# halide/Halide

Hardware: AMD Instinct MI355X
Metric: megapixels/sec local_laplacian 8-level fp32 4K (higher is better)
Workload: dtype f32; 1 GPU; apps/local_laplacian J=8 levels=8 alpha=1/7 beta=1, u16 RGB planar 3840x2160; distinct_frames_per_gpu=8, lut_cached=True, streams_per_gpu=4, frame_scheduling=4 frame-queue streams, boundary=C ABI local_laplacian(halide_buffer_t*,int32,float,float,halide_buffer_t*), rccl_ranks=1, parallelism=frames sharded over 1 GPU(s), no data-path collective

## Files before the change

halide_amd/csrc/hlmi_internal.h:

```cpp
#pragma once

#include <hip/hip_runtime.h>
#include <mutex>
#include <stdarg.h>
#include <stdint.h>
#include <stdio.h>
#include <string.h>
#include <type_traits>

#include "hlmi_pipelines.h"
#include "hlmi_runtime.h"

namespace hlmi {

int report(void *uc, int code, const char *fmt, ...) __attribute__((format(printf, 3, 4)));
int hip_failed(void *uc, hipError_t e, const char *what);

#define HLMI_HIP(uc, call)                                           \
    do {                                                             \
        hipError_t e__ = (call);                                     \
        if (e__ != hipSuccess) return ::hlmi::hip_failed(uc, e__, #call); \
    } while (0)

constexpr uint32_t type_abi(int code, int bits) { return (uint32_t)code | ((uint32_t)bits << 8); }
constexpr uint32_t T_U8 = type_abi(1, 8), T_U16 = type_abi(1, 16), T_I16 = type_abi(0, 16),
                   T_I32 = type_abi(0, 32), T_F32 = type_abi(2, 32);
inline uint32_t buf_type_abi(const halide_buffer_t *b) {
    uint32_t v;
    memcpy(&v, &b->type, 4);
    return v;
}
const char *type_name(uint32_t abi, char tmp[16]);

struct BufArg {
    const char *name;
    halide_buffer_t *buf;
    uint32_t type;
    int dims;
    bool is_output;
};

int check_not_null(void *uc, const BufArg *args, int n);
bool any_bounds_query(const BufArg *args, int n);
int check_type_and_dims(void *uc, const BufArg *args, int n);
int check_shape(void *uc, const BufArg &a);
int check_covers(void *uc, const BufArg &a, int d, int req_min, int req_extent);
int check_equal(void *uc, const char *what, int val, const char *expect_what, int expect);
int checks_done(void *uc);
void answer_query(halide_buffer_t *buf, const int *mins, const int *extents);

struct DeviceCtx {
    int device = -1;
    hipStream_t stream = nullptr;
    std::unique_lock<std::recursive_mutex> call_lock;
};
int acquire_device(void *uc, DeviceCtx *ctx, bool lock = true);
int get_workspace(void *uc, const DeviceCtx &ctx, size_t bytes, void **ptr);

int input_to_device(void *uc, const DeviceCtx &ctx, const BufArg &a);
int output_on_device(void *uc, const DeviceCtx &ctx, const BufArg &a);
void mark_output_written(halide_buffer_t *buf);
uint64_t buffer_version(const halide_buffer_t *buf);
int stream_cu_count(int device, hipStream_t stream);

inline bool buffer_is_real(const halide_buffer_t *b) { return !(b->host == nullptr && b->device == 0); }
inline bool buffer_has_shape(const halide_buffer_t *b) {
    for (int d = 0; d < b->dimensions; d++)
        if (b->dim[d].extent <= 0) return false;
    return b->dimensions > 0;
}
inline bool buffer_known(const halide_buffer_t *b) { return buffer_is_real(b) || buffer_has_shape(b); }

inline bool stream_is_special(hipStream_t s) { return s == nullptr || s == hipStreamLegacy || s == hipStreamPerThread; }
inline hipError_t record_done(hipEvent_t ev, hipStream_t producer) {
    if (stream_is_special(producer)) return hipStreamSynchronize(producer == hipStreamLegacy ? nullptr : producer);
    return hipEventRecord(ev, producer);
}
inline hipError_t wait_done(hipStream_t consumer, hipEvent_t ev) {
    if (stream_is_special(consumer)) return hipEventSynchronize(ev);
    return hipStreamWaitEvent(consumer, ev, 0);
}
inline hipStream_t event_stream(hipStream_t s) { return s == hipStreamLegacy ? nullptr : s; }

template<typename T>
inline T *dev_ptr(const halide_buffer_t *b) { return reinterpret_cast<T *>((uintptr_t)b->device); }

constexpr int DERIVED_SLOTS = 8, DERIVED_READERS = 4;
constexpr size_t DERIVED_KEY_BYTES = 96;
struct DerivedEntry {
    unsigned char key[DERIVED_KEY_BYTES];
    size_t key_bytes = 0;
    int device = -1;
    size_t bytes = 0;
    void *ptr = nullptr;
    hipStream_t stream = nullptr;
    hipEvent_t ready = nullptr;
    struct Reader {
        hipStream_t s = nullptr;
        hipEvent_t done = nullptr;
        bool live = false;
    } readers[DERIVED_READERS];
    bool overflow = false;
    int pins = 0;
    uint64_t used = 0;
};
struct DerivedCache {
    const int capacity;
    std::mutex mu;
    DerivedEntry slots[DERIVED_SLOTS];
    uint64_t clock = 0;
    explicit DerivedCache(int n) : capacity(n) {}
};
struct DerivedUse {
    void *ptr = nullptr;
    bool fill = true;
    void filled(hipStream_t s);
// ... 57 lines not shown
```

halide_amd/csrc/local_laplacian.hip:

```cpp
#include "hlmi_device_math.h"
#include "hlmi_internal.h"

#include <atomic>
#include <mutex>
#include <optional>
#include <stdlib.h>
#include <string.h>
#include <type_traits>

using namespace hlmi;

namespace {

constexpr int J = 8;
constexpr int MAX_K = 32;
constexpr int STRIP = 126;
constexpr int KCH = 8;
constexpr int D0_THREADS = 256;

struct Level {
    int lox, loy;
    int w, h;
    int ws;
    size_t ps;
// ... 604 lines not shown
    prep_row(rd, p1);
    load_row(rc, 2 * T0 + 3);
    load_row(rd, 2 * T0 + 4);
    LL_PROBE_T(pt2);
    for (int T = T0; T <= T1; T += 2) {
        const bool first = EXCH && T == T0;
        step(std::integral_constant<int, 0>{}, T, p0, p1, p2, p3, a, b, a2, b2, first && publish ? pub_mine : nullptr);
        step(std::integral_constant<int, 1>{}, T + 1, p2, p3, p0, p1, a2, b2, a, b,
             first && publish ? pub_mine + (KCH + 1) * 64 : nullptr);
        if (first) __syncthreads();
#if HLMI_LL_PROBE
        if (first) { LL_PROBE_T(pt3); pr_3 = pt3; }
#endif
    }
    LL_PROBE_T(pt4);
    LL_PROBE_ADD(0, pt1 - pt0); LL_PROBE_ADD(1, 1); LL_PROBE_ADD(2, pt2 - pt1); LL_PROBE_ADD(3, pr_3 - pt2);
    LL_PROBE_ADD(16, pr_a - pr_a0); LL_PROBE_ADD(17, pr_a0 - pt1);
    LL_PROBE_ADD(4, pt4 - pt2); LL_PROBE_ADD(5, (T1 - T0 + 1)); LL_PROBE_ADD(6, pt4 - pt0);
    if (EXCH && !self_halo) {
        float *d2 = p.g2 + (size_t)(B - p.loy2) * p.ws2 + off2;
#pragma unroll
        for (int k = 0; k <= KCH; k++) {
            const float2 sa = st2[(2 * k) * 64], sb = st2[(2 * k + 1) * 64];
            const float2 c = pub_next[k * 64], d = pub_next[(KCH + 1 + k) * 64];
            const float rx = dev::mad(3.0f, sb.x + c.x, sa.x) + d.x, ry = dev::mad(3.0f, sb.y + c.y, sa.y) + d.y;
            float o;
            if (ODD1) {
                const float nx = lane_next(rx), ny = lane_next(ry);
                o = down4_tail(rx, ry, nx, ny);
            } else {
                const float py = lane_prev(ry), nx = lane_next(rx);
                o = down4_tail(py, rx, ry, nx);
            }
            if (st2_ok) d2[(size_t)k * p.ps2] = o;
        }
    }
    };
    if (edge_wave) walk(std::true_type{});
    else walk(std::false_type{});
}

struct D01EArgs {
    D01Args d;
    float *outl0;
    int oy0, oh;
    unsigned nsx_magic;
};
typedef float f2 __attribute__((ext_vector_type(2)));
__device__ __forceinline__ f2 f2s(float v) { return f2{v, v}; }
__device__ __forceinline__ f2 fma2(f2 a, f2 b, f2 c) { return __builtin_elementwise_fma(a, b, c); }
__device__ __forceinline__ f2 mad_2(f2 a, f2 b, f2 c) { return dev::CANON_FMA ? fma2(a, b, c) : a * b + c; }
__device__ __forceinline__ f2 mad2_2(f2 a, f2 b, f2 c, f2 d) { return dev::CANON_FMA ? fma2(a, b, c * d) : a * b + c * d; }

template<bool ODD0, bool ODD1, bool B1, bool EXCH, bool NT>
__global__ __launch_bounds__(D0_THREADS, 2) void ll_down01e(D01EArgs pe, Geometry gm, Levels lev) {
    const D01Args &p = pe.d;
    LL_RESIDENCY(0);
    extern __shared__ float slut[];
    for (int i = threadIdx.x; i <= 2 * gm.half; i += D0_THREADS) slut[i] = p.lut_g[i];
    __syncthreads();
    const int wave = __builtin_amdgcn_readfirstlane(threadIdx.x >> 6);
    const int lane = threadIdx.x & 63;
    int sx, A, B;
    bool self_halo = true;
    bool publish = false;
    if (EXCH) {
        const int wg = xcd_block();
        const int gy = pe.nsx_magic ? (int)__umulhi((unsigned)wg, pe.nsx_magic) : wg;
        sx = wg - gy * p.nsx;
        const int GA = p.loy2 + gy * p.rows_base + min(gy, p.rows_rem);
        const int GB = GA + p.rows_base + (gy < p.rows_rem ? 1 : 0) - 1;
        const int n = (GB - GA + 1 + 1 + 3) >> 2;
        A = GA + wave * n, B = min(A + n - 1, GB);
        if (A > GB) {
            __syncthreads();
            return;
        }
        self_halo = !(wave < 3 && A + n <= GB);
        publish = wave > 0;
    } else {
        const int unit = xcd_block() * (D0_THREADS / 64) + wave;
        if (unit >= p.nunits) return;
        sx = p.nsy_magic ? (int)__umulhi((unsigned)unit, p.nsy_magic) : unit;
        const int sy = unit - sx * p.nsy;
        A = p.loy2 + sy * p.rows_base + min(sy, p.rows_rem);
        B = A + p.rows_base + (sy < p.rows_rem ? 1 : 0) - 1;
    }
    const int P = p.Pbase + 2 * p.S2 * sx + 2 * lane;
    const int q0 = ODD0 ? 2 * P - 1 : 2 * P - 2;
    const int iw = gm.ix1 - gm.ix0 + 1, ih = gm.iy1 - gm.iy0;
    const QuadSel qs = quad_sel(q0 - gm.ix0, iw);
    int xo[4];
#pragma unroll
    for (int i = 0; i < 4; i++) xo[i] = qs.oq + qs.sel[i];
    const bool edge_wave = __any(!qs.plain);
    const int T0 = 2 * A - 1, T1 = self_halo ? 2 * B + 2 : 2 * B;
    const int Ts0 = max(EXCH ? 2 * A - 1 : 2 * A, p.loy1), Ts1 = min(EXCH ? 2 * B : 2 * B + 1, p.loy1 + p.h1 - 1);
    const int off1 = P - p.so1;
    const bool st1_ok = lane < p.S2 && off1 >= 0 && off1 < p.w1;
    const int X2 = ODD1 ? (P + 1) >> 1 : P >> 1;
    const int off2 = X2 - p.so2;
    const bool st2_ok = (ODD1 ? lane < p.S2 : (lane >= 1 && lane <= p.S2)) && off2 >= 0 && off2 < p.w2;
    const bool em_ok = lane >= 1 && lane <= p.S2 && q0 >= gm.ix0 && q0 + 3 <= gm.ix1;
    float *const em_col = pe.outl0 + (q0 - gm.ix0);
    f2 *st2 = reinterpret_cast<f2 *>(slut + ((2 * gm.half + 2) & ~1)) + wave * D01_STATE + lane;
    f2 *pub_all = reinterpret_cast<f2 *>(slut + ((2 * gm.half + 2) & ~1)) + (D0_THREADS / 64) * D01_STATE + lane;
    f2 *pub_mine = pub_all + (wave - 1) * D01_STATE, *pub_next = pub_all + wave * D01_STATE;
    const int lbase = gm.half - 256 * (KCH - 1);
    float level[KCH];
#pragma unroll
    for (int kk = 0; kk < KCH; kk++) {
        level[kk] = lev.v[kk];
        asm volatile("" : "+v"(level[kk]));
    }
    auto walk = [&](auto edge_tag) {
    constexpr bool EDGE = decltype(edge_tag)::value;
    auto load_row = [&](Raw &r, int y_abs) {
        const uint16_t *rp = p.in + (long)(dev::clampi(y_abs - gm.iy0, 0, ih)) * p.in_sy;
        load_raw<true, NT>(r, rp, p.co0, p.co1, p.co2, qs.oq, xo);
    };
    auto u16s = [&](const ushort4 &c, uint16_t (&o)[4]) {
        const uint2 w = __builtin_bit_cast(uint2, c);
        o[0] = (uint16_t)(w.x & 0xffffu), o[1] = (uint16_t)(w.x >> 16);
        o[2] = (uint16_t)(w.y & 0xffffu), o[3] = (uint16_t)(w.y >> 16);
    };
    struct Row {
        f2 g[2];
        int l[4];
    };
    auto prep_row = [&](const Raw &r, Row &o) {
        uint16_t rr[4], gg[4], bb[4];
        u16s(r.c0, rr), u16s(r.c1, gg), u16s(r.c2, bb);
        constexpr float s = (float)(1.0 / 65535.0);
        constexpr float C0 = (float)((double)s * (double)0.299f), C1 = (float)((double)s * (double)0.587f),
                        C2 = (float)((double)s * (double)0.114f);
#pragma unroll
        for (int h = 0; h < 2; h++) {
            const f2 fr = {(float)rr[h], (float)rr[h + 2]}, fg = {(float)gg[h], (float)gg[h + 2]}, fb = {(float)bb[h], (float)bb[h + 2]};
            o.g[h] = mad_2(fb, f2s(C2), mad2_2(fr, f2s(C0), fg, f2s(C1)));
        }
        if (EDGE) {
            const float g0 = o.g[0].x, g1v = o.g[1].x, g2v = o.g[0].y, g3 = o.g[1].y;
            o.g[0].x = pick4(g0, g1v, g2v, g3, qs.sel[0]), o.g[1].x = pick4(g0, g1v, g2v, g3, qs.sel[1]);
            o.g[0].y = pick4(g0, g1v, g2v, g3, qs.sel[2]), o.g[1].y = pick4(g0, g1v, g2v, g3, qs.sel[3]);
        }
#pragma unroll
        for (int h = 0; h < 2; h++) {
            const f2 t = (o.g[h] * gm.Km1) * 256.0f;
            o.l[h] = (min((int)t.x, gm.half) + lbase) * 4;
            o.l[h + 2] = (min((int)t.y, gm.half) + lbase) * 4;
        }
#pragma unroll
        for (int i = 0; i < 4; i++) asm volatile("" : "+v"(o.l[i]));
    };
    auto lut_issue = [&](int kk, const Row &r0, const Row &r1, f2 (&dst)[4]) {
        auto rd = [&](int l) {
            return *reinterpret_cast<const float *>(reinterpret_cast<const char *>(slut) + l + 1024 * (KCH - 1 - kk));
        };
        dst[0].x = rd(r0.l[0]), dst[1].x = rd(r0.l[1]), dst[0].y = rd(r0.l[2]), dst[1].y = rd(r0.l[3]);
        dst[2].x = rd(r1.l[0]), dst[3].x = rd(r1.l[1]), dst[2].y = rd(r1.l[2]), dst[3].y = rd(r1.l[3]);
// ... 236 lines not shown
            em_wait(eg[0], after3), eo[0] = em_arith(n0, 0, eg[0], row_odd);
            __builtin_amdgcn_sched_barrier(0);
            em_gather(n1, 0, rowP, rowT, fg[0]);
            __builtin_amdgcn_sched_barrier(0);
            em_wait(eg[1], after3), eo[1] = em_arith(n0, 1, eg[1], row_odd);
            __builtin_amdgcn_sched_barrier(0);
            em_gather(n1, 1, rowP, rowT, fg[1]);
            __builtin_amdgcn_sched_barrier(0);
            em_wait(eg[2], after3), eo[2] = em_arith(n0, 2, eg[2], row_odd);
            __builtin_amdgcn_sched_barrier(0);
            em_gather(n1, 2, rowP, rowT, fg[2]);
            __builtin_amdgcn_sched_barrier(0);
            em_wait(eg[3], after3), eo[3] = em_arith(n0, 3, eg[3], row_odd);
            __builtin_amdgcn_sched_barrier(0);
            em_gather(n1, 3, rowP, rowT, fg[3]);
            __builtin_amdgcn_sched_barrier(0);
            em_wait(fg[0], after3), ee[0] = em_arith(n1, 0, fg[0], row_even);
            em_wait(fg[1], after2), ee[1] = em_arith(n1, 1, fg[1], row_even);
            em_wait(fg[2], after1), ee[2] = em_arith(n1, 2, fg[2], row_even);
            em_wait(fg[3], after0), ee[3] = em_arith(n1, 3, fg[3], row_even);
        }
        asm volatile("" ::: "memory");
        __builtin_amdgcn_sched_barrier(0);
        LL_PROBE_T(ps2);
        prep_row(rc, n0);
        prep_row(rd, n1);
        __builtin_amdgcn_sched_barrier(0);
        if (st1_row && st1_ok) {
            float *drow = p.g1 + (size_t)(T - p.loy1) * p.ws1 + off1;
            *reinterpret_cast<float2 *>(drow) = s0;
            *reinterpret_cast<float2 *>(drow + p.ps1) = s1;
            *reinterpret_cast<f2 *>(drow + (size_t)KCH * p.ps1) = sK;
        }
        if (em_rows) {
            emit_store(2 * T - 1, eo);
            emit_store(2 * T, ee);
        }
        __builtin_amdgcn_sched_barrier(0);
        if (T + 1 < T1) {
            load_row(rc, 2 * T + 5);
            load_row(rd, 2 * T + 6);
        }
        __builtin_amdgcn_sched_barrier(0);
#if HLMI_LL_PROBE
        LL_PROBE_T(ps3);
        pr_planes += ps1 - ps0, pr_emit += ps2 - ps1, pr_prep += ps3 - ps2, pr_steps += 1;
#endif
    };
    Row p0, p1, p2, p3;
    prep_row(rc, p0);
    prep_row(rd, p1);
    load_row(rc, 2 * T0 + 3);
    load_row(rd, 2 * T0 + 4);
    for (int T = T0; T <= T1; T += 2) {
        const bool first = EXCH && T == T0;
        step(std::integral_constant<int, 0>{}, T, p0, p1, p2, p3, a, b, a2, b2, first && publish ? pub_mine : nullptr);
        step(std::integral_constant<int, 1>{}, T + 1, p2, p3, p0, p1, a2, b2, a, b, first && publish ? pub_mine + 64 : nullptr);
        if (first) __syncthreads();
    }
#if HLMI_LL_PROBE
    LL_PROBE_T(pe1);
#endif
    if (EXCH && !self_halo) {
        float *d2 = p.g2 + (size_t)(B - p.loy2) * p.ws2 + off2;
#pragma unroll
        for (int k = 0; k <= KCH; k++) {
            const f2 sa = st2[(2 * k) * 64], sb = st2[(2 * k + 1) * 64];
            const f2 c = pub_next[(2 * k) * 64], d = pub_next[(2 * k + 1) * 64];
            const f2 r = mad_2(f2s(3.0f), sb + c, sa) + d;
            float o;
            if (ODD1) {
                const float nx = lane_next(r.x), ny = lane_next(r.y);
                o = down4_tail(r.x, r.y, nx, ny);
            } else {
                const float py = lane_prev(r.y), nx = lane_next(r.x);
                o = down4_tail(py, r.x, r.y, nx);
            }
            if (st2_ok) d2[(size_t)k * p.ps2] = o;
        }
        {
            float eo[4], ee[4];
            emit_row(p2, pub_next, st2 + 64, eo, row_odd);
            emit_row(p3, st2 + 64, pub_next, ee, row_even);
            emit_store(4 * B + 1, eo);
            emit_store(4 * B + 2, ee);
        }
    }
#if HLMI_LL_PROBE
    LL_PROBE_T(pe2);
    LL_PROBE_ADD(27, __builtin_readcyclecounter() - pc0);
    LL_PROBE_ADD(28, pe2 - pe0);
    LL_PROBE_ADD(20, pr_planes); LL_PROBE_ADD(21, pr_emit); LL_PROBE_ADD(22, pr_prep); LL_PROBE_ADD(23, pr_steps);
    LL_PROBE_ADD(24, 1); LL_PROBE_ADD(25, pe1 - pe0); LL_PROBE_ADD(26, pe2 - pe1);
#endif
    };
    if (edge_wave) walk(std::true_type{});
    else walk(std::false_type{});
}

struct StripArgs {
    const float *src;
    int slox, sloy, sw, sh, sws;
    size_t sps;
    float *dst;
    int Xs, dloy, dw, dh, dws;
    size_t dps;
    int nsx, nsy, nunits;
};
template<bool ODD>
__device__ __forceinline__ void down_strip_unit(const StripArgs &a, int unit, int lane) {
    const int sy = unit % a.nsy, rest = unit / a.nsy, sx = rest % a.nsx, plane = rest / a.nsx;
    const int off = STRIP * sx + 2 * lane;
    const int P = a.Xs + off;
    const QuadSel qs = quad_sel((ODD ? 2 * P - 1 : 2 * P - 2) - a.slox, a.sw);
    const bool edge_wave = __any(!qs.plain);
    const bool store_ok = (lane < 63) && (off < a.dw);
    const int t0 = (int)((long)sy * a.dh / a.nsy), t1 = (int)((long)(sy + 1) * a.dh / a.nsy) - 1;
    const float *sp = a.src + (size_t)plane * a.sps + qs.oq;
    float *dp = a.dst + (size_t)plane * a.dps + off;
    auto row = [&](int y_abs) -> float4 {
        float4 v = *reinterpret_cast<const float4 *>(sp + (size_t)dev::clampi(y_abs - a.sloy, 0, a.sh - 1) * a.sws);
        if (edge_wave) {
            v = make_float4(pick4(v.x, v.y, v.z, v.w, qs.sel[0]), pick4(v.x, v.y, v.z, v.w, qs.sel[1]),
                            pick4(v.x, v.y, v.z, v.w, qs.sel[2]), pick4(v.x, v.y, v.z, v.w, qs.sel[3]));
        }
        return v;
    };
    const int T0 = a.dloy + t0;
    float4 ra = row(2 * T0 - 1), rb = row(2 * T0), rc = row(2 * T0 + 1), rd = row(2 * T0 + 2);
    for (int t = t0; t <= t1; t++) {
        const int T = a.dloy + t;
        float4 nc = rc, nd = rd;
        if (t < t1) {
            nc = row(2 * T + 3);
            nd = row(2 * T + 4);
        }
// ... 881 lines not shown
const halide_scalar_value_t est_one = [] { halide_scalar_value_t v{}; v.u.f32 = 1.0f; return v; }();
const halide_type_t ty_u16 = {(decltype(halide_type_t::code))1, 16, 0};
const halide_type_t ty_i32 = {(decltype(halide_type_t::code))0, 32, 0};
const halide_type_t ty_f32 = {(decltype(halide_type_t::code))2, 32, 0};
const halide_filter_argument_t ll_args[5] = {
    {"input", halide_argument_kind_input_buffer, 3, ty_u16, nullptr, nullptr, nullptr, nullptr, buf_est},
    {"levels", halide_argument_kind_input_scalar, 0, ty_i32, nullptr, nullptr, nullptr, &est_levels, nullptr},
    {"alpha", halide_argument_kind_input_scalar, 0, ty_f32, nullptr, nullptr, nullptr, &est_one, nullptr},
    {"beta", halide_argument_kind_input_scalar, 0, ty_f32, nullptr, nullptr, nullptr, &est_one, nullptr},
    {"output", halide_argument_kind_output_buffer, 3, ty_u16, nullptr, nullptr, nullptr, nullptr, buf_est},
};
const halide_filter_metadata_t ll_md = {1, 5, ll_args, kTargetString, "local_laplacian"};

struct LlSwitches {
    std::optional<int> fuse_from, upchain_from, ru, units0, no_vec, emit, nt, fuse_up2, d01_exch, d01_pad_lds, no_lut_cache;
};
LlSwitches ll_switches() {
    auto get = [](const char *name) -> std::optional<int> {
        const char *e = getenv(name);
        if (e && *e) return atoi(e);
        return std::nullopt;
    };
    LlSwitches s;
    s.fuse_from = get("HLMI_LL_FUSE_FROM"), s.upchain_from = get("HLMI_LL_UPCHAIN_FROM");
    s.ru = get("HLMI_LL_RU"), s.units0 = get("HLMI_LL_UNITS0"), s.no_vec = get("HLMI_LL_NO_VEC");
    s.emit = get("HLMI_LL_EMIT"), s.nt = get("HLMI_LL_NT"), s.fuse_up2 = get("HLMI_LL_FUSE_UP2");
    s.d01_exch = get("HLMI_LL_D01_EXCH"), s.d01_pad_lds = get("HLMI_LL_D01_PAD_LDS"), s.no_lut_cache = get("HLMI_LL_NO_LUT_CACHE");
    return s;
}

int dev_clamp_ru(int ru) { return ru < 1 ? 1 : (ru > 300 ? 300 : ru); }

struct PairGeom {
    int S2;
    int Pbase;
    int nsx;
};
struct LlPlan {
    Geometry gm;
    Level lv[J];
    size_t off_g[J], off_out[J], off_l0, ws_floats;
    Up0Args u0;
    int nlut;
    int S, SU;
    int up_low;
    bool lut_cache;
    bool lut_lds;
    bool vec_frame;
    bool vec_in;
    bool b1;
    bool fast, fuse1, fuse2, emit, nt;
    bool d01;
    bool strip2;
    struct { PairGeom pg; bool exch; int nsy, nunits; size_t lds; } d0;
    struct { PairGeom pg; int nsy, nunits; } s2;
    int units_strip;
    size_t up0_lds;
};

struct LlBuffers {
    float *lut, *outl0;
    float *g[J], *outg[J];
};

PairGeom pair_geom(const Level &d, const Level &e) {
    PairGeom g;
    g.S2 = (d.odd || e.odd) ? 62 : 61;
    const int lim = e.odd ? 2 * e.lox - 1 : 2 * e.lox - 2;
    g.Pbase = min(d.lox, lim);
    const int hi1 = d.lox + d.w - 1, hi2 = e.lox + e.w - 1;
    const int x2_first = e.odd ? (g.Pbase + 1) / 2 + 0 : g.Pbase / 2 + 1;
    g.nsx = max((hi2 - x2_first + g.S2) / g.S2, (hi1 - g.Pbase + 2 * g.S2) / (2 * g.S2));
    return g;
}

void ll_plan(LlPlan &pl, const halide_buffer_t *input, const halide_buffer_t *output, int levels, float beta, const LlSwitches &sw,
             int stream_cus, int device_cus) {
    Up0Args &p = pl.u0;
    const int ow = p.ow = output->dim[0].extent, oh = p.oh = output->dim[1].extent, nc = p.nc = output->dim[2].extent;
    Geometry &gm = pl.gm;
    gm.K = levels;
    gm.half = (levels - 1) * 256;
    gm.Km1 = (float)(levels - 1);
    gm.inv_Km1 = 1.0f / gm.Km1;
    gm.ix0 = input->dim[0].min, gm.ix1 = gm.ix0 + input->dim[0].extent - 1;
    gm.iy0 = input->dim[1].min, gm.iy1 = gm.iy0 + input->dim[1].extent - 1;
    const int ic0 = input->dim[2].min, ic1 = ic0 + input->dim[2].extent - 1, iw = gm.ix1 - gm.ix0 + 1;

    Level *lv = pl.lv;
    int lox = gm.ix0, hix = gm.ix1, loy = gm.iy0, hiy = gm.iy1, so = gm.ix0;
    int rx0 = output->dim[0].min, rx1 = rx0 + ow - 1, ry0 = output->dim[1].min, ry1 = ry0 + oh - 1;
    size_t ws_floats = (size_t)(2 * gm.half + 1 + 63) & ~(size_t)63;
    for (int j = 0; j < J; j++) {
        Level &L = lv[j];
        L.lox = so, L.loy = loy, L.w = hix - so + 1, L.h = hiy - loy + 1;
        L.ws = (L.w + 3) & ~3;
        L.ps = ((size_t)L.ws * L.h + 3) & ~(size_t)3;
        L.rx0 = rx0, L.rx1 = rx1, L.ry0 = ry0, L.ry1 = ry1;
        if (j >= 1) {
            pl.off_g[j] = ws_floats;
            ws_floats += ((size_t)(levels + 1) * L.ps + 63) & ~(size_t)63;
            pl.off_out[j] = ws_floats;
            ws_floats += (L.ps + 63) & ~(size_t)63;
        }
        const bool odd = (so & 1) != 0;
        const int par = odd ? (floor_div(so + 1, 2) & 1) : ((floor_div(so, 2) + 1) & 1);
        lox = floor_div(lox - 2, 2), hix = floor_div(hix + 2, 2);
        loy = floor_div(loy - 2, 2), hiy = floor_div(hiy + 2, 2);
        so = lox - ((lox - par) & 1);
        if (j + 1 < J) {
            lv[j + 1].odd = odd;
            lv[j + 1].nsx = (hix - so + 1 + STRIP - 1) / STRIP;
        }
        rx0 = floor_div(rx0 - 1, 2), rx1 = floor_div(rx1 + 1, 2);
        ry0 = floor_div(ry0 - 1, 2), ry1 = floor_div(ry1 + 1, 2);
    }
    p.in = dev_ptr<uint16_t>(input), p.out = dev_ptr<uint16_t>(output);
    const uintptr_t din = (uintptr_t)p.in, dout = (uintptr_t)p.out;
    const long in_sy = p.in_sy = input->dim[1].stride, in_sc = input->dim[2].stride;
    const long out_sy = p.out_sy = output->dim[1].stride, out_sc = p.out_sc = output->dim[2].stride;
    p.ox0 = output->dim[0].min, p.oy0 = output->dim[1].min;
    p.beta = beta, pl.b1 = (beta == 1.0f);
    const int oc0 = output->dim[2].min;
    bool same = (nc == 3);
    for (int ch = 0; ch < 3; ch++) {
        p.gco[ch] = (long)((ch < ic0 ? ic0 : (ch > ic1 ? ic1 : ch)) - ic0) * in_sc;
        p.cco[ch] = ch < nc ? (long)(oc0 + ch - ic0) * in_sc : 0;
        if (p.cco[ch] != p.gco[ch]) same = false;
    }
    p.same_ch = same ? 1 : 0;
// ... 10 lines not shown
        const int v = sw.upchain_from.value_or(S == 4 ? 3 : 0);
        return (v >= 1 && v <= J - 2) ? v : S;
    }();
    const bool partitioned = stream_cus < device_cus;
    bool vec_frame = (din % 4 == 0) && (dout % 4 == 0) && in_sy % 2 == 0 && out_sy % 2 == 0 && out_sc % 2 == 0 &&
                     ((p.ox0 - gm.ix0) % 2 == 0) && !sw.no_vec.value_or(0);
    for (int ch = 0; ch < 3; ch++) vec_frame = vec_frame && p.gco[ch] % 2 == 0 && p.cco[ch] % 2 == 0;
    pl.vec_frame = vec_frame;
    const bool vec_in = pl.vec_in = (din % 8 == 0) && in_sy % 4 == 0 && p.gco[0] % 4 == 0 && p.gco[1] % 4 == 0 && p.gco[2] % 4 == 0 &&
                                    iw % 4 == 0 && !sw.no_vec.value_or(0);
    const bool fast = pl.fast = vec_frame && same && nc == 3 && (ow & 1) == 0 && (p.ox0 & 1) == 0 &&
                                (double)(levels + 1) * (4.0 * (double)lv[1].ps) < 4.0e9;
    const bool fuse1 = pl.fuse1 = fast && SU >= 2;
    const bool d01 = pl.d01 = levels == KCH && lut_lds && vec_in;
    const bool emit = pl.emit = d01 && fast && fuse1 && lv[1].ws < (1 << 24) && sw.emit.value_or(1);
    const int RU = p.RU = dev_clamp_ru(sw.ru.value_or(emit ? (partitioned ? 32 : 8) : fuse1 ? (partitioned ? 32 : 16) : 8));
    pl.nt = sw.nt.value_or(partitioned ? 1 : 0) != 0;
    pl.fuse2 = emit && SU >= 3 && SU < J && sw.fuse_up2.value_or(1);
    pl.up_low = fuse1 ? (pl.fuse2 ? 3 : 2) : 1;
    pl.strip2 = d01 && S == 4;

    pl.off_l0 = ws_floats;
    if (emit) ws_floats += ((size_t)iw * (size_t)oh + 63) & ~(size_t)63;
    pl.ws_floats = ws_floats;

    constexpr int WPB = D0_THREADS / 64;
    if (!d01) {
        const Level &d = lv[1];
        const int target = sw.units0.value_or(8 * device_cus);
        pl.d0.nsy = max(1, min(max(target / d.nsx, (d.h + 63) / 64), max(1, d.h / 2)));
        pl.d0.nunits = d.nsx * pl.d0.nsy;
        pl.d0.lds = (lut_lds ? sizeof(float) * ((nlut + 1) & ~1) : 0) + sizeof(float2) * D0_THREADS * (KCH + 1);
    } else {
        const Level &e = lv[2];
        const PairGeom pg = pl.d0.pg = pair_geom(lv[1], e);
        const int target2 = sw.units0.value_or(emit && partitioned ? 10 * stream_cus : 8 * device_cus);
        bool exch = sw.d01_exch.value_or(1) != 0;
        int nwy = 0;
        auto ceil_div = [](int x, int y) { return (x + y - 1) / y; };
        if (exch) {
            const int nwy_max = max(1, target2 / (WPB * pg.nsx));
            const int n = max(2, (ceil_div(e.h, nwy_max) + 1 + 3) / 4);
            nwy = ceil_div(e.h, 4 * n - 1);
            exch = e.h / nwy >= 4;
        }
        pl.d0.exch = exch;
        if (exch) {
            pl.d0.nsy = nwy;
            pl.d0.nunits = pg.nsx * nwy * WPB;
        } else {
            pl.d0.nsy = max(1, min(max(target2 / pg.nsx, (e.h + 31) / 32), e.h));
            pl.d0.nunits = pg.nsx * pl.d0.nsy;
        }
        size_t sh2 = sizeof(float) * ((nlut + 1) & ~1) + sizeof(float2) * D01_STATE * (WPB + (exch ? WPB - 1 : 0));
        const int pad = sw.d01_pad_lds.value_or(emit && partitioned ? -1 : 0);
        constexpr size_t kHalfCuLds = 160 * 1024 / 2;
        if (pad < 0) sh2 = max(sh2, kHalfCuLds + 2048);
        else sh2 += (size_t)pad;
        pl.d0.lds = sh2;
    }
    if (pl.strip2) {
        pl.s2.pg = pair_geom(lv[3], lv[4]);
        pl.s2.nsy = (lv[4].h + S2_RPU - 1) / S2_RPU;
        pl.s2.nunits = (levels + 1) * pl.s2.pg.nsx * pl.s2.nsy;
    }
    pl.units_strip = 16 * device_cus;
    pl.up0_lds = emit   ? sizeof(float) * ((size_t)U0_TS * (RU + 2) + (size_t)U0H_T2 * (RU / 2 + 4))
                 : fast ? lut_sh + (fuse1 ? ((lut_lds && (nlut & 1)) ? 4 : 0) + sizeof(float) * U0_TS * (RU + 2) : 0)
                        : lut_sh;
}

struct LlLastCall {
    LlPlan pl;
    LlBuffers b;
    hipStream_t stream;
    bool out1_pending;
    bool out2_pending;
};
thread_local LlLastCall t_dbg = {};

StripArgs strip_args(const LlPlan &pl, const LlBuffers &b, int j) {
    const Level &sl = pl.lv[j], &d = pl.lv[j + 1];
    const int cols = d.nsx * (pl.gm.K + 1);
    StripArgs a;
    a.src = b.g[j], a.slox = sl.lox, a.sloy = sl.loy, a.sw = sl.w, a.sh = sl.h, a.sws = sl.ws, a.sps = sl.ps;
    a.dst = b.g[j + 1], a.Xs = d.lox, a.dloy = d.loy, a.dw = d.w, a.dh = d.h, a.dws = d.ws, a.dps = d.ps;
    a.nsx = d.nsx;
    a.nsy = max(1, min(max(pl.units_strip / cols, (d.h + 31) / 32), max(1, d.h / 2)));
    a.nunits = cols * a.nsy;
    return a;
}
CoarseArgs coarse_args(const LlPlan &pl, const LlBuffers &b, int from) {
    CoarseArgs ca;
    for (int dl = 0; from + dl < J; dl++) {
        const Level &L = pl.lv[from + dl];
        DevLevel &D = ca.lv[dl];
        D.g = b.g[from + dl], D.out = b.outg[from + dl], D.lox = L.lox, D.loy = L.loy, D.w = L.w, D.h = L.h, D.ws = L.ws, D.ps = (unsigned)L.ps;
        D.rx0 = L.rx0, D.ry0 = L.ry0, D.rw = L.rx1 - L.rx0 + 1, D.rh = L.ry1 - L.ry0 + 1;
    }
    ca.K = pl.gm.K, ca.Km1 = pl.gm.Km1;
    return ca;
}
UpArgs up_args(const LlPlan &pl, const LlBuffers &b, int j) {
    const Level &a = pl.lv[j], &c = pl.lv[j + 1];
    UpArgs u;
    u.g = b.g[j], u.ws = a.ws, u.ps = a.ps, u.lox = a.lox, u.loy = a.loy, u.gc = b.g[j + 1], u.outc = b.outg[j + 1], u.cws = c.ws, u.cps = c.ps;
    u.clox = c.lox, u.cloy = c.loy, u.rx0 = a.rx0, u.ry0 = a.ry0, u.rw = a.rx1 - a.rx0 + 1, u.rh = a.ry1 - a.ry0 + 1;
    u.K = pl.gm.K, u.Km1 = pl.gm.Km1, u.out = b.outg[j];
    return u;
}

// ... 4 lines not shown
static_assert(sizeof(LutKey) <= DERIVED_KEY_BYTES, "key does not fit an entry");
DerivedCache g_luts(8);


int ll_stage_table(void *uc, const DeviceCtx &ctx, const LlPlan &pl, float alpha, LlBuffers &b, DerivedUse &use) {
    const int nlut = pl.nlut;
    LutKey key;
    memset(&key, 0, sizeof key);
    key.device = ctx.device, key.levels = pl.gm.K;
    memcpy(&key.alpha_bits, &alpha, 4);
    int r = derived_acquire(uc, ctx, g_luts, &key, sizeof key, sizeof(float) * ((size_t)nlut + 64), pl.lut_cache, &use);
    if (r) return r;
    if (use.ptr) b.lut = (float *)use.ptr;
    if (use.fill) {
        HLMI_LAUNCH(uc, "ll_remap_lut", ctx.stream, ll_remap_lut, dim3((nlut + 255) / 256), dim3(256), 0, b.lut, pl.gm.half, alpha);
        use.filled(ctx.stream);
    }
    return 0;
}

int ll_stage_down0(void *uc, const LlPlan &pl, const LlBuffers &b, hipStream_t st) {
    const Geometry &gm = pl.gm;
    const Up0Args &f = pl.u0;
    const Level &d = pl.lv[1], &e = pl.lv[2];
    const int levels = gm.K, iw = gm.ix1 - gm.ix0 + 1;
    Levels lev;
    for (int k = 0; k < MAX_K; k++) lev.v[k] = (float)k * gm.inv_Km1;
    constexpr int WPB = D0_THREADS / 64;
    dim3 block(D0_THREADS);
    const double d0_bytes = 6.0 * iw * (gm.iy1 - gm.iy0 + 1) + 4.0 * (levels + 1) * d.w * d.h;
    if (!pl.d01) {
        dim3 grid((pl.d0.nunits + WPB - 1) / WPB);
        timing_note_bytes(d0_bytes);
        return with_flags([&](auto O, auto V, auto L, auto B) -> int {
            HLMI_LAUNCH(uc, "ll_down0", st, (ll_down0<O.value, V.value, L.value, B.value>), grid, block, pl.d0.lds, f.in, f.in_sy,
                        f.gco[0], f.gco[1], f.gco[2], gm, lev, f.beta, b.lut, b.g[1], d.lox, d.loy, d.w, d.h, d.ws, d.ps, d.nsx,
                        pl.d0.nsy, pl.d0.nunits);
            return 0;
        }, d.odd, pl.vec_in, pl.lut_lds, pl.b1);
    }
    D01Args a;
    a.in = f.in, a.in_sy = f.in_sy, a.co0 = f.gco[0], a.co1 = f.gco[1], a.co2 = f.gco[2], a.beta = f.beta, a.lut_g = b.lut;
    a.g1 = b.g[1], a.so1 = d.lox, a.loy1 = d.loy, a.w1 = d.w, a.h1 = d.h, a.ws1 = d.ws, a.ps1 = d.ps;
    a.g2 = b.g[2], a.so2 = e.lox, a.loy2 = e.loy, a.w2 = e.w, a.h2 = e.h, a.ws2 = e.ws, a.ps2 = e.ps;
    a.S2 = pl.d0.pg.S2, a.Pbase = pl.d0.pg.Pbase, a.nsx = pl.d0.pg.nsx, a.nsy = pl.d0.nsy, a.nunits = pl.d0.nunits;
    a.nsy_magic = a.nsy == 1 ? 0u : (unsigned)((1ull << 32) / (unsigned)a.nsy + 1ull);
    a.rows_base = e.h / a.nsy, a.rows_rem = e.h % a.nsy;
    dim3 grid((a.nunits + WPB - 1) / WPB);
    if (pl.emit) {
        timing_note_bytes(6.0 * iw * (gm.iy1 - gm.iy0 + 1) + 4.0 * iw * f.oh + 4.0 * 3.0 * d.w * d.h + 4.0 * (levels + 1) * e.w * e.h);
        D01EArgs ae;
        ae.d = a, ae.outl0 = b.outl0, ae.oy0 = f.oy0, ae.oh = f.oh;
        ae.nsx_magic = a.nsx == 1 ? 0u : (unsigned)((1ull << 32) / (unsigned)a.nsx + 1ull);
        return with_flags([&](auto O0, auto O1, auto B, auto EX, auto NT) -> int {
            HLMI_LAUNCH(uc, "ll_down01", st, (ll_down01e<O0.value, O1.value, B.value, EX.value, NT.value>), grid, block, pl.d0.lds, ae, gm, lev);
            return 0;
        }, d.odd, e.odd, pl.b1, pl.d0.exch, pl.nt);
    }
    timing_note_bytes(d0_bytes + 4.0 * (levels + 1) * e.w * e.h);
    return with_flags([&](auto O0, auto O1, auto B, auto EX) -> int {
        HLMI_LAUNCH(uc, "ll_down01", st, (ll_down01f<O0.value, O1.value, B.value, EX.value>), grid, block, pl.d0.lds, a, gm, lev);
        return 0;
    }, d.odd, e.odd, pl.b1, pl.d0.exch);
}

int ll_stage_down_rest(void *uc, const LlPlan &pl, const LlBuffers &b, hipStream_t st) {
    const Level *lv = pl.lv;
    const int levels = pl.gm.K, S = pl.S;
    if (pl.strip2) {
        const Level &sl = lv[2], &d = lv[3], &e = lv[4];
        Strip2Args a;
        a.src = b.g[2], a.slox = sl.lox, a.sloy = sl.loy, a.sw = sl.w, a.sh = sl.h, a.sws = sl.ws, a.sps = sl.ps;
        a.g1 = b.g[3], a.so1 = d.lox, a.loy1 = d.loy, a.w1 = d.w, a.h1 = d.h, a.ws1 = d.ws, a.ps1 = d.ps;
        a.g2 = b.g[4], a.so2 = e.lox, a.loy2 = e.loy, a.w2 = e.w, a.h2 = e.h, a.ws2 = e.ws, a.ps2 = e.ps;
        a.S2 = pl.s2.pg.S2, a.Pbase = pl.s2.pg.Pbase, a.nsx = pl.s2.pg.nsx, a.nsy = pl.s2.nsy, a.nunits = pl.s2.nunits;
        timing_note_bytes(4.0 * (levels + 1) * ((double)sl.w * sl.h + (double)d.w * d.h + (double)e.w * e.h));
        dim3 grid((a.nunits + 3) / 4), block(256);
        if (int r = with_flags([&](auto O0, auto O1) -> int {
                HLMI_LAUNCH(uc, "ll_down_strip2:2", st, (ll_down_strip2<O0.value, O1.value>), grid, block, 0, a);
                return 0;
            }, d.odd, e.odd)) return r;
    }
    for (int j = 1; j + 1 < J; j++) {
        if (pl.strip2 && (j == 2 || j == 3)) continue;
        if (j == S) {
            const CoarseArgs ca = coarse_args(pl, b, S);
            long total = 0;
            for (int dl = 1; S + dl < J; dl++) total += (long)(levels + 1) * lv[S + dl].w * lv[S + dl].h;
            const int ntx = (lv[J - 1].w + DM_T - 1) / DM_T, nty = (lv[J - 1].h + DM_T - 1) / DM_T;
            dim3 grid((unsigned)(ntx * nty * (levels + 1))), block(256);
            char nm[32];
            snprintf(nm, sizeof nm, "ll_down_multi:%d", S);
            timing_note_bytes(4.0 * ((double)(levels + 1) * lv[S].w * lv[S].h + (double)total));
            if (J - 1 - S == 4) HLMI_LAUNCH(uc, nm, st, (ll_down_multi<4>), grid, block, 0, ca, ntx, nty);
            else if (J - 1 - S == 3) HLMI_LAUNCH(uc, nm, st, (ll_down_multi<3>), grid, block, 0, ca, ntx, nty);
            else if (J - 1 - S == 2) HLMI_LAUNCH(uc, nm, st, (ll_down_multi<2>), grid, block, 0, ca, ntx, nty);
            else HLMI_LAUNCH(uc, nm, st, (ll_down_multi<1>), grid, block, 0, ca, ntx, nty);
            break;
        }
        if (j == 1 && pl.d01) continue;
        const StripArgs sa = strip_args(pl, b, j);
        dim3 grid((sa.nunits + 3) / 4), block(256);
        char nm[32];
        snprintf(nm, sizeof nm, "ll_down_strip:%d", j);
        timing_note_bytes(4.0 * (levels + 1) * ((double)lv[j].w * lv[j].h + (double)lv[j + 1].w * lv[j + 1].h));
        if (int r = with_flags([&](auto O) -> int {
// ... 65 lines not shown
    if (pl.fast) {
        return with_flags([&](auto L, auto B, auto F) -> int {
            HLMI_LAUNCH(uc, "ll_up0", st, (ll_up0f<L.value, B.value, F.value>), grid, block, pl.up0_lds, p, gm);
            return 0;
        }, pl.lut_lds, pl.b1, pl.fuse1);
    }
    return with_flags([&](auto V, auto L) -> int {
        HLMI_LAUNCH(uc, "ll_up0", st, (ll_up0<V.value, L.value>), grid, block, pl.up0_lds, p, gm);
        return 0;
    }, pl.vec_frame, pl.lut_lds);
}

}

extern "C" int local_laplacian(halide_buffer_t *input, int32_t levels, float alpha, float beta, halide_buffer_t *output) {
    void *uc = nullptr;
    const LlSwitches sw = ll_switches();
    BufArg args[2] = {{"input", input, T_U16, 3, false}, {"output", output, T_U16, 3, true}};
    int r = check_not_null(uc, args, 2);
    if (r) return r;
    if ((r = check_type_and_dims(uc, args, 2))) return r;
    if (any_bounds_query(args, 2)) {
        int mins[3], ext[3];
        for (int d = 0; d < 3; d++) mins[d] = output->dim[d].min, ext[d] = output->dim[d].extent;
        answer_query(input, mins, ext);
        answer_query(output, mins, ext);
        return 0;
    }
    if ((r = check_shape(uc, args[0])) || (r = check_shape(uc, args[1]))) return r;
    for (int d = 0; d < 3; d++) {
        if ((r = check_covers(uc, args[0], d, output->dim[d].min, output->dim[d].extent))) return r;
    }
    if (levels < 2) {
        return report(uc, halide_error_code_param_too_small, "Parameter levels is %d but must be at least 2", levels);
    }
    if (levels > (1 << 20)) {
        return report(uc, halide_error_code_param_too_large, "Parameter levels is %d but must be at most %d", levels, 1 << 20);
    }
    const int nc = output->dim[2].extent;
    if (nc > 3) {
        return report(uc, halide_error_code_constraint_violated, "Output buffer output has %d channels, at most 3 supported", nc);
    }

    DeviceCtx ctx;
    if ((r = acquire_device(uc, &ctx))) return r;
    if ((r = input_to_device(uc, ctx, args[0]))) return r;
    if ((r = output_on_device(uc, ctx, args[1]))) return r;
    if (output->dim[0].extent == 0 || output->dim[1].extent == 0 || nc == 0) {
        mark_output_written(output);
        return 0;
    }

    LlPlan pl;
    ll_plan(pl, input, output, levels, beta, sw, stream_cu_count(ctx.device, ctx.stream), stream_cu_count(ctx.device, nullptr));

    void *ws = nullptr;
    if ((r = get_workspace(uc, ctx, pl.ws_floats * sizeof(float), &ws))) return r;
    float *wsf = (float *)ws;
    LlBuffers b;
    b.lut = wsf, b.outl0 = wsf + pl.off_l0;
    b.g[0] = b.outg[0] = nullptr;
    for (int j = 1; j < J; j++) b.g[j] = wsf + pl.off_g[j], b.outg[j] = wsf + pl.off_out[j];
    t_dbg.pl = pl, t_dbg.b = b, t_dbg.stream = ctx.stream;
    t_dbg.out1_pending = pl.fuse1, t_dbg.out2_pending = pl.fuse2;

    hipStream_t st = ctx.stream;
    DerivedUse table;
    if ((r = ll_stage_table(uc, ctx, pl, alpha, b, table)) || (r = ll_stage_down0(uc, pl, b, st)) || (r = ll_stage_down_rest(uc, pl, b, st)) ||
        (r = ll_stage_up_coarse(uc, pl, b, st)) || (r = ll_stage_up0(uc, pl, b, st))) {
        return r;
    }
    table.done(st);
    mark_output_written(output);
    return 0;
}

extern "C" int local_laplacian_argv(void **a) {
    return local_laplacian((halide_buffer_t *)a[0], *(int32_t *)a[1], *(float *)a[2], *(float *)a[3],
                           (halide_buffer_t *)a[4]);
}
extern "C" const halide_filter_metadata_t *local_laplacian_metadata(void) { return &ll_md; }
extern "C" int local_laplacian_auto_schedule(halide_buffer_t *input, int32_t levels, float alpha, float beta,
                                             halide_buffer_t *output) {
    return local_laplacian(input, levels, alpha, beta, output);
}

extern "C" int hlmi_debug_ll_probe(unsigned long long *out32) {
#if HLMI_LL_PROBE
    if (hipDeviceSynchronize() != hipSuccess) return -1;
    if (hipMemcpyFromSymbol(out32, HIP_SYMBOL(g_probe), sizeof(unsigned long long) * 32) != hipSuccess) return -1;
    unsigned long long zero[32] = {};
    if (hipMemcpyToSymbol(HIP_SYMBOL(g_probe), zero, sizeof zero) != hipSuccess) return -1;
    return 1;
#else
    (void)out32;
    return 0;
#endif
}

extern "C" int hlmi_debug_ll_residency(unsigned long long *out16) {
#if HLMI_LL_RESIDENCY
    if (hipDeviceSynchronize() != hipSuccess) return -1;
    if (hipMemcpyFromSymbol(out16, HIP_SYMBOL(g_res_hist), sizeof(unsigned long long) * 16) != hipSuccess) return -1;
    unsigned long long zero[16] = {};
    if (hipMemcpyToSymbol(HIP_SYMBOL(g_res_hist), zero, sizeof zero) != hipSuccess) return -1;
    return 1;
#else
// ... 67 lines not shown
```

halide_amd/csrc/runtime.cpp:

```cpp
#include <atomic>
#include <map>
#include <mutex>
#include <tuple>
#include <string>
#include <unordered_map>
#include <vector>

#include <dlfcn.h>
#include <stdlib.h>

#include "hlmi_internal.h"
#include "hlmi_device_math.h"

namespace hlmi {

const char *const kTargetString = "x86-64-linux-hip-gfx950";

static void default_error_handler(void *, const char *msg) {
    fprintf(stderr, "Error: %s\n", msg);
    fflush(stderr);
    abort();
}
static void default_print(void *, const char *msg) { fputs(msg, stderr); }
static void *default_malloc(void *, size_t x) {
// ... 348 lines not shown
    }
}

static Owned *find_owned_locked(uint64_t handle, int *dev_out) {
    int n = device_count_locked();
    for (int d = 0; d < n; d++) {
        auto &m = g_dev[d].owned;
        auto it = m.upper_bound(handle);
        if (it == m.begin()) continue;
        --it;
        if (handle >= it->first && handle < it->first + it->second.bytes) {
            if (dev_out) *dev_out = d;
            return &it->second;
        }
    }
    return nullptr;
}

static int note_use(void *uc, const DeviceCtx &ctx, uint64_t handle, const char *name, bool written = false) {
    std::lock_guard<std::mutex> lock(g_mu);
    int dev;
    Owned *o = find_owned_locked(handle, &dev);
    if (!o) return 0;
    if (dev != ctx.device) {
        return report(uc, halide_error_code_incompatible_device_interface,
                      "Buffer %s lives on GPU device %d but this call runs on device %d (halide_set_gpu_device)", name, dev,
                      ctx.device);
    }
    order_after_locked(dev, ctx.stream, o->last_stream);
    o->last_stream = ctx.stream;
    if (written) o->version = ++g_version_counter;
    return 0;
}

static std::map<std::tuple<int, int, int, int>, hipStream_t> g_part_streams;
static std::unordered_map<hipStream_t, int> g_part_cus;

int stream_cu_count(int device, hipStream_t stream) {
    {
        std::lock_guard<std::mutex> lock(g_mu);
        auto it = g_part_cus.find(stream);
        if (it != g_part_cus.end()) return it->second;
    }
    static const int share = [] { const char *e = getenv("HLMI_STREAM_SHARE"); return e && atoi(e) > 1 ? atoi(e) : 1; }();
    static std::atomic<int> cached[64];
    int c = cached[device & 63].load();
    if (c <= 0) {
        if (hipDeviceGetAttribute(&c, hipDeviceAttributeMultiprocessorCount, device) != hipSuccess || c <= 0) c = 256;
        cached[device & 63].store(c);
    }
    return stream ? c / share : c;
}

static bool stream_outlives_entries(int device, hipStream_t s) {
    if (stream_is_special(s)) return true;
    std::lock_guard<std::mutex> lock(g_mu);
    return s == g_dev[device].stream || g_part_cus.count(s) != 0;
}

static void wait_for_users(DerivedEntry &e, hipStream_t consumer) {
    bool sync_all = e.overflow || consumer == nullptr;
    if (!sync_all && e.stream != consumer) {
        if (!stream_outlives_entries(e.device, e.stream)) sync_all = true;
        else if (e.ready && wait_done(consumer, e.ready) != hipSuccess) (void)hipGetLastError(), sync_all = true;
    }
    for (auto &r : e.readers) {
        if (r.live && !sync_all && r.s != consumer) {
            bool ok = stream_outlives_entries(e.device, r.s) && (r.done || hipEventCreateWithFlags(&r.done, hipEventDisableTiming) == hipSuccess);
            ok = ok && record_done(r.done, r.s) == hipSuccess && wait_done(consumer, r.done) == hipSuccess;
            if (!ok) {
                (void)hipGetLastError();
                sync_all = true;
            }
        }
        r.live = false;
    }
    if (sync_all) {
        int cur = -1;
        (void)hipGetDevice(&cur);
        if (cur != e.device && e.device >= 0) (void)hipSetDevice(e.device);
        (void)hipDeviceSynchronize();
        if (cur >= 0 && cur != e.device) (void)hipSetDevice(cur);
        (void)hipGetLastError();
    }
    e.overflow = false;
}

void DerivedUse::filled(hipStream_t s) {
    if (entry) (void)record_done(entry->ready, s);
    fill = false;
}

void DerivedUse::done(hipStream_t s) {
    if (entry) {
        if (!lock.owns_lock()) lock = std::unique_lock<std::mutex>(cache->mu);
        if (pinned) entry->pins--, pinned = false;
        DerivedEntry::Reader *slot = nullptr;
        for (auto &r : entry->readers) {
            if (r.live && r.s == s) slot = &r;
        }
        if (!slot) {
            for (auto &r : entry->readers) {
                if (!r.live) { slot = &r; break; }
            }
        }
        if (slot) slot->s = s, slot->live = true;
// ... 972 lines not shown
```

Baseline: 115,700 Mpx/s.

## Exchange down01 seam rows through registers and size LDS padding from device query

Adds a SEAMR variant of the fused down01 kernel where, in partitioned emit mode, each wave copies the neighbouring wave's seam state into registers after the first step, instead of keeping a separate publish area in LDS. This removes the (WPB-1) publish slots from shared memory and drops the artificial padding that forced one workgroup per CU, so the kernel is sized to its real LDS need and launched with launch_bounds min-blocks 1. The half-CU padding now comes from the queried per-CU LDS size instead of a hardcoded 160 KiB. Costs include more registers per thread, an extra barrier, and a write-back of the seam into the wave's own state before emitting rows.

```diff
diff --git a/halide_amd/csrc/hlmi_internal.h b/halide_amd/csrc/hlmi_internal.h
--- a/halide_amd/csrc/hlmi_internal.h
+++ b/halide_amd/csrc/hlmi_internal.h
@@ -62,6 +62,7 @@
 void mark_output_written(halide_buffer_t *buf);
 uint64_t buffer_version(const halide_buffer_t *buf);
 int stream_cu_count(int device, hipStream_t stream);
+size_t device_cu_lds(int device);
 
 inline bool buffer_is_real(const halide_buffer_t *b) { return !(b->host == nullptr && b->device == 0); }
 inline bool buffer_has_shape(const halide_buffer_t *b) {
diff --git a/halide_amd/csrc/local_laplacian.hip b/halide_amd/csrc/local_laplacian.hip
--- a/halide_amd/csrc/local_laplacian.hip
+++ b/halide_amd/csrc/local_laplacian.hip
@@ -680,8 +680,9 @@
 __device__ __forceinline__ f2 mad_2(f2 a, f2 b, f2 c) { return dev::CANON_FMA ? fma2(a, b, c) : a * b + c; }
 __device__ __forceinline__ f2 mad2_2(f2 a, f2 b, f2 c, f2 d) { return dev::CANON_FMA ? fma2(a, b, c * d) : a * b + c * d; }
 
-template<bool ODD0, bool ODD1, bool B1, bool EXCH, bool NT>
-__global__ __launch_bounds__(D0_THREADS, 2) void ll_down01e(D01EArgs pe, Geometry gm, Levels lev) {
+template<bool ODD0, bool ODD1, bool B1, bool EXCH, bool NT, bool SEAMR = false>
+__global__ __launch_bounds__(D0_THREADS, SEAMR ? 1 : 2) void ll_down01e(D01EArgs pe, Geometry gm, Levels lev) {
+    static_assert(EXCH || !SEAMR, "seam rows are exchanged by EXCH workgroups only");
     const D01Args &p = pe.d;
     LL_RESIDENCY(0);
     extern __shared__ float slut[];
@@ -702,10 +703,11 @@
         A = GA + wave * n, B = min(A + n - 1, GB);
         if (A > GB) {
             __syncthreads();
+            if (SEAMR) __syncthreads();
             return;
         }
         self_halo = !(wave < 3 && A + n <= GB);
-        publish = wave > 0;
+        publish = wave > 0 && !SEAMR;
     } else {
         const int unit = xcd_block() * (D0_THREADS / 64) + wave;
         if (unit >= p.nunits) return;
@@ -734,6 +736,7 @@
     f2 *st2 = reinterpret_cast<f2 *>(slut + ((2 * gm.half + 2) & ~1)) + wave * D01_STATE + lane;
     f2 *pub_all = reinterpret_cast<f2 *>(slut + ((2 * gm.half + 2) & ~1)) + (D0_THREADS / 64) * D01_STATE + lane;
     f2 *pub_mine = pub_all + (wave - 1) * D01_STATE, *pub_next = pub_all + wave * D01_STATE;
+    const f2 *st2_below = st2 + D01_STATE;
     const int lbase = gm.half - 256 * (KCH - 1);
     float level[KCH];
 #pragma unroll
@@ -1076,11 +1079,21 @@
     prep_row(rd, p1);
     load_row(rc, 2 * T0 + 3);
     load_row(rd, 2 * T0 + 4);
+    f2 seam_c[KCH + 1], seam_d[KCH + 1];
+#pragma unroll
+    for (int k = 0; k <= KCH; k++) seam_c[k] = seam_d[k] = f2s(0.0f);
     for (int T = T0; T <= T1; T += 2) {
         const bool first = EXCH && T == T0;
         step(std::integral_constant<int, 0>{}, T, p0, p1, p2, p3, a, b, a2, b2, first && publish ? pub_mine : nullptr);
         step(std::integral_constant<int, 1>{}, T + 1, p2, p3, p0, p1, a2, b2, a, b, first && publish ? pub_mine + 64 : nullptr);
         if (first) __syncthreads();
+        if (SEAMR && first) {
+            if (!self_halo) {
+#pragma unroll
+                for (int k = 0; k <= KCH; k++) seam_c[k] = st2_below[(2 * k) * 64], seam_d[k] = st2_below[(2 * k + 1) * 64];
+            }
+            __syncthreads();
+        }
     }
 #if HLMI_LL_PROBE
     LL_PROBE_T(pe1);
@@ -1090,7 +1103,7 @@
 #pragma unroll
         for (int k = 0; k <= KCH; k++) {
             const f2 sa = st2[(2 * k) * 64], sb = st2[(2 * k + 1) * 64];
-            const f2 c = pub_next[(2 * k) * 64], d = pub_next[(2 * k + 1) * 64];
+            const f2 c = SEAMR ? seam_c[k] : pub_next[(2 * k) * 64], d = SEAMR ? seam_d[k] : pub_next[(2 * k + 1) * 64];
             const f2 r = mad_2(f2s(3.0f), sb + c, sa) + d;
             float o;
             if (ODD1) {
@@ -1102,10 +1115,19 @@
             }
             if (st2_ok) d2[(size_t)k * p.ps2] = o;
         }
+        const f2 *row_c = pub_next;
+        if (SEAMR) {
+            asm volatile("" ::: "memory");
+#pragma unroll
+            for (int k = 0; k <= KCH; k++) st2[(2 * k) * 64] = seam_c[k];
+            asm volatile("" ::: "memory");
+            __builtin_amdgcn_wave_barrier();
+            row_c = st2;
+        }
         {
             float eo[4], ee[4];
-            emit_row(p2, pub_next, st2 + 64, eo, row_odd);
-            emit_row(p3, st2 + 64, pub_next, ee, row_even);
+            emit_row(p2, row_c, st2 + 64, eo, row_odd);
+            emit_row(p3, st2 + 64, row_c, ee, row_even);
             emit_store(4 * B + 1, eo);
             emit_store(4 * B + 2, ee);
         }
@@ -2093,7 +2115,7 @@
     bool fast, fuse1, fuse2, emit, nt;
     bool d01;
     bool strip2;
-    struct { PairGeom pg; bool exch; int nsy, nunits; size_t lds; } d0;
+    struct { PairGeom pg; bool exch, seam_regs; int nsy, nunits; size_t lds; } d0;
     struct { PairGeom pg; int nsy, nunits; } s2;
     int units_strip;
     size_t up0_lds;
@@ -2116,7 +2138,7 @@
 }
 
 void ll_plan(LlPlan &pl, const halide_buffer_t *input, const halide_buffer_t *output, int levels, float beta, const LlSwitches &sw,
-             int stream_cus, int device_cus) {
+             int stream_cus, int device_cus, size_t cu_lds) {
     Up0Args &p = pl.u0;
     const int ow = p.ow = output->dim[0].extent, oh = p.oh = output->dim[1].extent, nc = p.nc = output->dim[2].extent;
     Geometry &gm = pl.gm;
@@ -2233,11 +2255,11 @@
             pl.d0.nsy = max(1, min(max(target2 / pg.nsx, (e.h + 31) / 32), e.h));
             pl.d0.nunits = pg.nsx * pl.d0.nsy;
         }
-        size_t sh2 = sizeof(float) * ((nlut + 1) & ~1) + sizeof(float2) * D01_STATE * (WPB + (exch ? WPB - 1 : 0));
         const int pad = sw.d01_pad_lds.value_or(emit && partitioned ? -1 : 0);
-        constexpr size_t kHalfCuLds = 160 * 1024 / 2;
-        if (pad < 0) sh2 = max(sh2, kHalfCuLds + 2048);
-        else sh2 += (size_t)pad;
+        const bool seam_regs = pl.d0.seam_regs = emit && partitioned && exch && pad < 0;
+        size_t sh2 = sizeof(float) * ((nlut + 1) & ~1) + sizeof(float2) * D01_STATE * (WPB + (exch && !seam_regs ? WPB - 1 : 0));
+        if (pad >= 0) sh2 += (size_t)pad;
+        else if (!seam_regs) sh2 = max(sh2, cu_lds / 2 + 2048);
         pl.d0.lds = sh2;
     }
     if (pl.strip2) {
@@ -2348,6 +2370,12 @@
         D01EArgs ae;
         ae.d = a, ae.outl0 = b.outl0, ae.oy0 = f.oy0, ae.oh = f.oh;
         ae.nsx_magic = a.nsx == 1 ? 0u : (unsigned)((1ull << 32) / (unsigned)a.nsx + 1ull);
+        if (pl.d0.seam_regs) {
+            return with_flags([&](auto O0, auto O1, auto B, auto NT) -> int {
+                HLMI_LAUNCH(uc, "ll_down01", st, (ll_down01e<O0.value, O1.value, B.value, true, NT.value, true>), grid, block, pl.d0.lds, ae, gm, lev);
+                return 0;
+            }, d.odd, e.odd, pl.b1, pl.nt);
+        }
         return with_flags([&](auto O0, auto O1, auto B, auto EX, auto NT) -> int {
             HLMI_LAUNCH(uc, "ll_down01", st, (ll_down01e<O0.value, O1.value, B.value, EX.value, NT.value>), grid, block, pl.d0.lds, ae, gm, lev);
             return 0;
@@ -2519,7 +2547,8 @@
     }
 
     LlPlan pl;
-    ll_plan(pl, input, output, levels, beta, sw, stream_cu_count(ctx.device, ctx.stream), stream_cu_count(ctx.device, nullptr));
+    ll_plan(pl, input, output, levels, beta, sw, stream_cu_count(ctx.device, ctx.stream), stream_cu_count(ctx.device, nullptr),
+            device_cu_lds(ctx.device));
 
     void *ws = nullptr;
     if ((r = get_workspace(uc, ctx, pl.ws_floats * sizeof(float), &ws))) return r;
diff --git a/halide_amd/csrc/runtime.cpp b/halide_amd/csrc/runtime.cpp
--- a/halide_amd/csrc/runtime.cpp
+++ b/halide_amd/csrc/runtime.cpp
@@ -424,6 +424,16 @@
     return stream ? c / share : c;
 }
 
+size_t device_cu_lds(int device) {
+    static std::atomic<int> cached[64];
+    int c = cached[device & 63].load();
+    if (c <= 0) {
+        if (hipDeviceGetAttribute(&c, hipDeviceAttributeMaxSharedMemoryPerMultiprocessor, device) != hipSuccess || c <= 0) c = 160 * 1024;
+        cached[device & 63].store(c);
+    }
+    return (size_t)c;
+}
+
 static bool stream_outlives_entries(int device, hipStream_t s) {
     if (stream_is_special(s)) return true;
     std::lock_guard<std::mutex> lock(g_mu);
```

Measured after the change: 113,900 Mpx/s. -1.5%, worse.
